# lcrekko/lq_mpc

Measured on AMD Instinct MI355X. Metric: MPC QP-steps/sec (batched systems) at n_x=4,n_u=2,N=10; 1/2/4/8 GPU, higher is better.
Workload: dtype f64

## Files before the change

### lq_mpc_amd/csrc/lqmpc_r16.hip

```cpp
#include <cstdio>
#include "lqmpc_r16_body.h"
#include "lqmpc_launch.h"

namespace lqmpc {

template <int NX, int NU, int N, int MODE, int LPI>
__global__ void __launch_bounds__(64, (R16Build<NX, NU, N, LPI>::WAVES)) lqmpc_r16_kernel(KParams p)
{
    using C = R16<NX, NU, N, LPI, (R16Build<NX, NU, N, LPI>::OCC == 2)>;
    __shared__ double lds_raw[C::IPW * C::INST];
    r16_body<NX, NU, N, MODE, LPI, R16Build<NX, NU, N, LPI>::OCC, (MODE == MODE_ROLLOUT && R16Build<NX, NU, N, LPI>::CHUNKS)>(p, lds_raw, (long long)blockIdx.x * C::IPW, p.Bsz);
}

template <int NX, int NU, int N, int LPI>
__global__ void __launch_bounds__(64, (R16Build<NX, NU, N, LPI>::WAVES)) lqmpc_r16_plan_kernel(KParams p)
{
    using C = R16<NX, NU, N, LPI, (R16Build<NX, NU, N, LPI>::OCC == 2)>;
    __shared__ double lds_raw[C::IPW * C::INST];
    r16_body<NX, NU, N, MODE_SOLVE, LPI, R16Build<NX, NU, N, LPI>::OCC, false, true>(p, lds_raw, (long long)blockIdx.x * C::IPW, p.Bsz);
}

template <int NX, int NU, int N, int LPI>
static void launch_r16_one(const KParams &p, hipStream_t stream)
{
    constexpr int IPW = 64 / LPI;
    const dim3 grid((unsigned)((p.Bsz + IPW - 1) / IPW));
    if (p.mode == MODE_SOLVE && p.Uplan) hipLaunchKernelGGL((lqmpc_r16_plan_kernel<NX, NU, N, LPI>), grid, dim3(64), 0, stream, p);
    else if (p.mode == MODE_SOLVE) hipLaunchKernelGGL((lqmpc_r16_kernel<NX, NU, N, MODE_SOLVE, LPI>), grid, dim3(64), 0, stream, p);
    else if (p.mode == MODE_MAXVN) hipLaunchKernelGGL((lqmpc_r16_kernel<NX, NU, N, MODE_MAXVN, LPI>), grid, dim3(64), 0, stream, p);
    else if (p.mode == MODE_SWEEP) hipLaunchKernelGGL((lqmpc_r16_kernel<NX, NU, N, MODE_SWEEP, LPI>), grid, dim3(64), 0, stream, p);
    else {
#ifdef LQMPC_R16_PROF
        long long z[36] = {0};
        (void)hipMemcpyToSymbol(HIP_SYMBOL(g_r16_prof), z, sizeof z);
#endif
        hipLaunchKernelGGL((lqmpc_r16_kernel<NX, NU, N, MODE_ROLLOUT, LPI>), grid, dim3(64), 0, stream, p);
#ifdef LQMPC_R16_PROF
        (void)hipStreamSynchronize(stream);
        (void)hipMemcpyFromSymbol(z, HIP_SYMBOL(g_r16_prof), sizeof z);
        fprintf(stderr, "r16 prof (block %d ticks): set-up on the matrix core %lld v_r %lld | rollout %lld\n", PROFBLK, z[5], z[6], z[7]);
        fprintf(stderr, "r16 prof (grid): waves %lld  set-up %.0f  total %.0f ticks/wave | free wave-steps %lld at %.0f ticks | busy wave-steps %lld at %.0f ticks, "
                "%.2f wave-iterations each (steps 1..T-1); %lld wave-iterations on the general (primal-capable) path in all\n", z[15], (double)z[13] / z[15], (double)z[14] / z[15], z[10], (double)z[8] / (z[10] ? z[10] : 1),
                z[11], (double)z[9] / (z[11] ? z[11] : 1), (double)z[12] / (z[11] ? z[11] : 1), z[16]);
        fprintf(stderr, "r16 prof (grid, ticks/wave): set-up on the matrix core %.0f v_r %.0f\n", (double)z[22] / z[15], (double)z[23] / z[15]);
        fprintf(stderr, "r16 prof (grid): %lld dual-only wave-iterations at %.0f ticks, %lld general at %.0f ticks\n", z[26], (double)z[24] / (z[26] ? z[26] : 1), z[16],
                (double)z[25] / (z[16] ? z[16] : 1));
        fprintf(stderr, "r16 prof (grid): step 0: %.0f ticks/wave, %.2f wave-iterations/wave, %.2f of them general; %lld of %lld wavefronts ever took the general (P-reading) path\n",
                (double)z[27] / z[15], (double)z[28] / z[15], (double)z[29] / z[15], z[30], z[15]);
        fprintf(stderr, "r16 prof (grid): chunks of iteration-free steps: %lld committed, %lld discarded with %lld steps computed for nothing (%.2f %% of the free wave-steps)\n",
                z[31], z[32], z[33], 100.0 * (double)z[33] / (z[10] ? z[10] : 1));
#endif
    }
}

#define R16E(NX, NU, N) {NX, NU, N, 16, "lqmpc_r16_kernel<" #NX "," #NU "," #N ">", launch_r16_one<NX, NU, N, 16>}
#define R64E(NX, NU, N) {NX, NU, N, 64, "lqmpc_r64_kernel<" #NX "," #NU "," #N ">", launch_r16_one<NX, NU, N, 64>}
static const ShapeEntry g_r16[] = {
    R16E(4, 2, 10),
    R16E(2, 1, 10),
    R16E(2, 1, 5), R16E(2, 1, 6), R16E(2, 1, 7), R16E(2, 1, 8), R16E(2, 1, 9),
    R16E(2, 1, 20), R16E(2, 1, 30),
    R64E(4, 2, 20),
};

// ... 22 lines not shown
```

### lq_mpc_amd/csrc/lqmpc_r16_body.h

```cpp
#pragma once
#include "lqmpc_wg_linalg.h"
#include "lqmpc_r16_setup.h"

namespace lqmpc {

using wg::ldsd;
using wg::ldsi;
using wg::rowb;
using wg::fmac_rowb;
using wg::fmac_rowb_self;
using wg::fmac_rowb4;
using wg::fmac_rowb_self4;
using wg::fmac_rowb_self2;
using wg::fmac_rowb_self3;
using wg::fmac_rowb_lanes4;
using wg::fmac_rowb_lanes4x2;
using wg::dpp_settle;

#ifdef LQMPC_R16_PROF
__device__ long long g_r16_prof[36];
#define RPROF(k) do { const long long now_ = clock64(); if (threadIdx.x == 0 && blockIdx.x == PROFBLK) g_r16_prof[k] += now_ - prof_t; if (k < 7) prof_ph[k] += now_ - prof_t; prof_t = clock64(); } while (0)
#define RPROF_START long long prof_t = clock64()
#define RPROF_ADD(k, v) do { if (threadIdx.x == 0) atomicAdd((unsigned long long *)&g_r16_prof[k], (unsigned long long)(v)); } while (0)
#ifndef PROFBLK
#define PROFBLK 0
#endif
#else
#define RPROF(k) do { } while (0)
#define RPROF_START do { } while (0)
#define RPROF_ADD(k, v) do { } while (0)
#endif

typedef unsigned long long mask_t;

template <int NX, int NU, int N, int LPI = 16, bool PACKED = false>
struct R16 {
    static constexpr int n = N * NU;
    static constexpr int RB = (n + LPI - 1) / LPI;
    static constexpr int IPW = 64 / LPI;
    static constexpr int CS = 4 * (((n + 1) / 2 + 3) / 4);
    static constexpr int LDW = n + 1;
    static constexpr int PK = PACKED ? n * (n + 1) / 2 : n * LDW;
    static constexpr int VEC = LPI * RB;
    static constexpr int oP = 0, oW = PK, oR = 2 * PK, oX = oR + VEC, oY = oX + VEC, oL = oY + VEC;
    static constexpr int oC = oL + CS / 2;
    static constexpr int CN0 = 3 * NX * NX + NU * NU + NX * NU;
    static constexpr int CN1 = (NX > NU ? NX : NU) * (2 * NX + 2 * NU);
    static constexpr int CN = CN0 > CN1 ? CN0 : CN1;
    static constexpr int oG = (NX > 8) ? oR : 0;
    static constexpr int SETUP = oG + n * NX;
    static constexpr int END = oC + CN + (CN & 1);
    static constexpr int oD = (END > SETUP) ? END : SETUP;
    static constexpr int INST = oD + 2;
    static constexpr int MAXIT = 12;
    static_assert(LPI == 16 || LPI == 64, "a DPP row or the whole wavefront");
    static_assert((n + 1) / 2 <= CS && n <= 64, "the smaller side must fit the gathered system");
};

template <int NX, int NU, int N, int LPI>
struct R16Build {
    static constexpr int OCC = ((LPI == 16 && N * NU > 10) || LPI == 64 || NX > 8) ? 2 : 1;
    static constexpr long long LDS_BYTES = (long long)(64 / LPI) * R16<NX, NU, N, LPI, (OCC == 2)>::INST * 8;
    static constexpr int WAVES = ((OCC == 2 || (N * NU <= 10 && LPI == 16)) && LDS_BYTES * 8 <= 160 * 1024) ? 2 : 1;
    static constexpr bool CHUNKS = NX == 4 && NU == 2 && ((LPI == 16 && N == 10) || (LPI == 64 && N == 20));
};

template <int LPI>
__device__ __forceinline__ mask_t iballot(bool c, int q)
{
    if constexpr (LPI == 16) return (__ballot(c) >> (16 * q)) & 0xFFFFull;
    else return __ballot(c);
}
template <int LPI>
__device__ __forceinline__ double ibcast(double x, int k)
{
    if constexpr (LPI == 16) return rowb(x, k);
    else return wg::rdlane(x, k);
}
template <int LPI>
__device__ __forceinline__ void ifmac_self4(double *acc, double y, int k)
{
    if constexpr (LPI == 16) fmac_rowb_self4(acc[0], acc[1], acc[2], acc[3], y, k);
    else {
#pragma unroll
        for (int e = 0; e < 4; ++e) acc[e] = __builtin_fma(wg::rdlane(acc[e], k), y, acc[e]);
    }
}
template <int LPI, int K, int CS>
__device__ __forceinline__ void ifmac_self_tail(double (&S)[CS], double &rhs, double g)
{
    constexpr int r = K % 4;
    if constexpr (LPI == 16) {
        if constexpr (r == 0) fmac_rowb_self4(S[K + 1], S[K + 2], S[K + 3], rhs, g, K);
        else if constexpr (r == 1) fmac_rowb_self3(S[K + 1], S[K + 2], rhs, g, K);
        else if constexpr (r == 2) fmac_rowb_self2(S[K + 1], rhs, g, K);
        else fmac_rowb_self(rhs, g, K);
    } else {
#pragma unroll
        for (int j = K + 1; j < 4 * (K / 4) + 4; ++j) S[j] = __builtin_fma(wg::rdlane(S[j], K), g, S[j]);
        rhs = __builtin_fma(wg::rdlane(rhs, K), g, rhs);
    }
}
template <int LPI>
__device__ __forceinline__ void isettle(double &x)
{
    if constexpr (LPI == 16) dpp_settle(x);
}
__device__ __forceinline__ int rowb_i(int x, int c)
{
    switch (c) {
#define LQMPC_X(C) case C: return __builtin_amdgcn_update_dpp(0, x, 0x150 + C, 0xF, 0xF, true);
        LQMPC_ROWB_CASES(LQMPC_X)
#undef LQMPC_X
    }
    return x;
}
__device__ __forceinline__ unsigned row_or(unsigned x)
{
    x |= (unsigned)__builtin_amdgcn_update_dpp(0, (int)x, 0x128, 0xF, 0xF, false);
    x |= (unsigned)__builtin_amdgcn_update_dpp(0, (int)x, 0x124, 0xF, 0xF, false);
    x |= (unsigned)__builtin_amdgcn_update_dpp(0, (int)x, 0x122, 0xF, 0xF, false);
    x |= (unsigned)__builtin_amdgcn_update_dpp(0, (int)x, 0x121, 0xF, 0xF, false);
    return x;
}
__device__ __forceinline__ unsigned row_umax(unsigned x)
{
    x = max(x, (unsigned)__builtin_amdgcn_update_dpp(0, (int)x, 0x128, 0xF, 0xF, false));
    x = max(x, (unsigned)__builtin_amdgcn_update_dpp(0, (int)x, 0x124, 0xF, 0xF, false));
    x = max(x, (unsigned)__builtin_amdgcn_update_dpp(0, (int)x, 0x122, 0xF, 0xF, false));
    x = max(x, (unsigned)__builtin_amdgcn_update_dpp(0, (int)x, 0x121, 0xF, 0xF, false));
    return x;
}

template <int NX, int NU, int N, int MODE, int LPI = 16, int OCC = 1, bool CHUNKS = false, bool PLAN = false>
__device__ __forceinline__ void r16_body(const KParams &p, double *lds_raw, long long slot0, long long slot_end)
{
    constexpr bool PACKED = (OCC == 2);
    using C = R16<NX, NU, N, LPI, PACKED>;
    constexpr int CS = C::CS;
    constexpr int n = C::n, RB = C::RB, LDW = C::LDW;
    constexpr int REC = NX * NX + NX * NU + NX;
    const int lane = threadIdx.x, q = lane / LPI, i = lane % LPI;
    ldsd *L = (ldsd *)lds_raw + q * C::INST;
    ldsd *Pp = L + C::oP, *Wp = L + C::oW, *rL = L + C::oR, *xL = L + C::oX, *yL = L + C::oY;
    ldsi *list = (ldsi *)(L + C::oL);
    const long long Bsz = p.Bsz;
    const long long b_raw = slot0 + q;
    const bool valid = b_raw < slot_end;
    const long long slot = valid ? b_raw : slot_end - 1;
    const long long b = p.perm ? (long long)p.perm[slot] : slot;
    const double *sh = p.sh;
    const mask_t nmask = (n == 64) ? ~0ull : ((1ull << n) - 1ull);

    int rw[RB], tri[RB];
    bool vrow[RB];
#pragma unroll
    for (int s = 0; s < RB; ++s) {
        rw[s] = i + LPI * s;
        tri[s] = rw[s] * (rw[s] + 1) / 2;
        vrow[s] = rw[s] < n;
    }

    auto ad = [&](int r, int tr, int j) -> int { if constexpr (PACKED) return (j <= r) ? tr + j : j * (j + 1) / 2 + r; else return r * LDW + j; };
    auto ad2 = [&](int a, int b2) -> int {
        if constexpr (PACKED) { const int hi = a > b2 ? a : b2, lo = a > b2 ? b2 : a; return hi * (hi + 1) / 2 + lo; }
        else return a * LDW + b2;
    };

    double G[RB][NX], vr[RB];
    constexpr bool CTL_F = MODE == MODE_CTL_FACTOR, CTL_S = MODE == MODE_CTL_STEP, CTL_R = MODE == MODE_CTL_ROLL;
    constexpr bool CTL_REC = CTL_S || CTL_R;
    using CR = CtlRecT<NX, NU, N>;
    constexpr bool LAZY_P = (LPI == 64 && !CTL_F) || CTL_REC;
    bool P_ready = !LAZY_P;
    bool W_ready = !CTL_REC;
    bool face_stays = false;
    auto tri_rc = [](int e, int &r, int &c) {
        r = (int)((__builtin_sqrtf(8.0f * (float)e + 1.0f) - 1.0f) * 0.5f);
        r = ((r + 1) * (r + 2) / 2 <= e) ? r + 1 : r;
        r = (r * (r + 1) / 2 > e) ? r - 1 : r;
        c = e - r * (r + 1) / 2;
    };
#ifdef LQMPC_NO_ROLL
    constexpr bool ROLL = false;
#else
    constexpr bool ROLL = LPI == 16 && NX <= 8 && N * ((NX + 3) / 4) <= 12 && MODE != MODE_MAXVN && !CTL_F && !CTL_REC;
#endif
    unsigned cold32[2] = {0u, 0u};
    bool cold_armed = false;
#ifdef LQMPC_R16_PROF
    const long long prof_t0 = clock64();
    int prof_wit = 0, prof_slow = 0, prof_fast = 0;
    long long prof_slowt = 0;
    long long prof_ph[8] = {0, 0, 0, 0, 0, 0, 0, 0};
#endif
    if constexpr (CTL_REC) {
        const double *rc = p.ctl_rec + b * p.ctl_stride;
#pragma unroll
        for (int s = 0; s < RB; ++s) {
            const int mr = vrow[s] ? rw[s] : 0;
#pragma unroll
            for (int a = 0; a < NX; ++a) G[s][a] = rc[CR::oG + mr * NX + a];
            vr[s] = vrow[s] ? rc[CR::oV + mr] : 0.0;
        }
    } else {
        RPROF_START;
        long long bg = b;
        ldsd *Lg = L;
        if constexpr (LPI == 16) {
            const int gq = (lane >> 2) & 3;
            const long long sraw = slot0 + gq, sl = sraw < slot_end ? sraw : slot_end - 1;
            bg = p.perm ? (long long)p.perm[sl] : sl;
            Lg = (ldsd *)lds_raw + gq * C::INST;
        }
        if constexpr (NX > 8) {
            static_assert(LPI == 16 && C::oG >= 2 * C::PK, "wide states: four instances per wavefront, G handed over behind P and W");
            r16_setup_wide<NX, NU, N, PACKED, RB>(setup_args(p), bg, Lg, C::oW, C::oG, C::oD);
#pragma unroll
            for (int s = 0; s < RB; ++s) {
#pragma unroll
                for (int a = 0; a < NX; ++a) {
                    const double x = L[C::oG + (vrow[s] ? rw[s] * NX + a : 0)];
                    G[s][a] = vrow[s] ? x : 0.0;
                }
            }
            __syncthreads();
        } else r16_setup_mfma<NX, NU, N, LPI, PACKED, RB, ROLL>(setup_args(p), bg, Lg, L, C::oW, C::oG, C::oD, G, roll_args(p), cold32[0], cold32[1]);
        if constexpr (!LAZY_P) r16_build_P<NX, NU, N, LPI, PACKED>(setup_args(p), bg, Lg, C::oP, C::oD);
        RPROF(5);
        const bool has_lin = p.has_lin != 0;
#pragma unroll
        for (int s = 0; s < RB; ++s) vr[s] = 0.0;
        if (has_lin) {
            if (p.has_ref) {
                double qr[RB];
#pragma unroll
                for (int s = 0; s < RB; ++s) qr[s] = 0.0;
                constexpr bool WIDE = NX > 8;
                double lam[NX], A2[WIDE ? 1 : NX][WIDE ? 1 : NX], B2[WIDE ? 1 : NX][WIDE ? 1 : NU];
                if constexpr (WIDE) {
                    const int ia = i < NX ? i : 0;
                    double Ac[NX], Bc[RB][NX];
#pragma unroll
                    for (int c = 0; c < NX; ++c) {
                        lam[c] = 0.0;
                        Ac[c] = p.rec ? p.rec[b * REC + c * NX + ia] : p.A[(long long)(c * NX + ia) * Bsz + b];
#pragma unroll
                        for (int s = 0; s < RB; ++s)
                            Bc[s][c] = p.rec ? p.rec[b * REC + NX * NX + c * NU + rw[s] % NU] : p.B[(long long)(c * NU + rw[s] % NU) * Bsz + b];
                    }
#pragma unroll 1
                    for (int r = N - 1; r >= 0; --r) {
                        const int oQ = (r < N - 1) ? p.so.Q : p.so.P;
                        double t = 0.0;
#pragma unroll
                        for (int c = 0; c < NX; ++c) t = __builtin_fma(sh[oQ + ia * NX + c], -sh[p.so.xref + c * N + r], t);
#pragma unroll
                        for (int c = 0; c < NX; ++c) t = __builtin_fma(Ac[c], lam[c], t);
                        yL[i] = t;
                        __syncthreads();
#pragma unroll
                        for (int a = 0; a < NX; ++a) lam[a] = yL[a];
                        __syncthreads();
#pragma unroll
                        for (int s = 0; s < RB; ++s) {
                            const int ui = rw[s] % NU;
                            double tk = 0.0;
#pragma unroll
                            for (int a = 0; a < NX; ++a) tk = __builtin_fma(Bc[s][a], lam[a], tk);
#pragma unroll
                            for (int j = 0; j < NU; ++j) tk = __builtin_fma(-sh[p.so.R + ui * NU + j], sh[p.so.uref + j * N + r], tk);
                            qr[s] = (vrow[s] && rw[s] / NU == r) ? 2.0 * tk : qr[s];
                        }
                    }
                } else {
#pragma unroll
                    for (int a = 0; a < NX; ++a) {
                        lam[a] = 0.0;
#pragma unroll
                        for (int c = 0; c < NX; ++c) A2[a][c] = p.rec ? p.rec[b * REC + a * NX + c] : p.A[(long long)(a * NX + c) * Bsz + b];
#pragma unroll
// ... 66 lines not shown
            }
        }
        RPROF(6);
    }
    if constexpr (CTL_F) {
        __syncthreads();
        const long long ir = p.ctl_idx ? (long long)p.ctl_idx[b] : b;
        if (valid && (unsigned long long)ir < (unsigned long long)p.ctl_n) {
            double *rc = p.ctl_rec + ir * p.ctl_stride;
            for (int e = i; e < NX * NX; e += LPI) rc[CR::oA + e] = p.A[(long long)e * Bsz + b];
            for (int e = i; e < NX * NU; e += LPI) rc[CR::oB + e] = p.B[(long long)e * Bsz + b];
#pragma unroll
            for (int s = 0; s < RB; ++s) {
                if (vrow[s]) {
#pragma unroll
                    for (int a = 0; a < NX; ++a) rc[CR::oG + rw[s] * NX + a] = G[s][a];
                    rc[CR::oV + rw[s]] = vr[s];
                }
            }
            for (int e = i; e < CR::tri; e += LPI) {
                int r, c;
                tri_rc(e, r, c);
                rc[CR::oW + e] = Wp[ad2(r, c)];
                rc[CR::oP + e] = Pp[ad2(r, c)];
            }
        }
        return;
    }
    auto ctl_fill = [&](ldsd *M, int off, bool on) {
        const double *src = p.ctl_rec + b * p.ctl_stride + off;
        constexpr int CNT = (CR::tri + LPI - 1) / LPI;
        double val[CNT];
#pragma unroll
        for (int k = 0; k < CNT; ++k) { const int e = i + LPI * k; val[k] = (on && e < CR::tri) ? src[e] : 0.0; }
#pragma unroll
        for (int k = 0; k < CNT; ++k) {
            const int e = i + LPI * k;
            if (on && e < CR::tri) {
                if constexpr (PACKED) M[e] = val[k];
                else { int r, c; tri_rc(e, r, c); M[r * LDW + c] = val[k]; M[c * LDW + r] = val[k]; }
            }
        }
        __syncthreads();
    };
    RPROF_START;
    RPROF_ADD(13, clock64() - prof_t0);

    long long bq = b;
    asm volatile("" : "+v"(bq));
    double h[RB], ctr[RB];
#pragma unroll
    for (int s = 0; s < RB; ++s) {
        const int k = rw[s] % NU;
        h[s] = vrow[s] ? 0.5 * (sh[p.so.ub + k] - sh[p.so.lb + k]) : 1.0;
        ctr[s] = vrow[s] ? 0.5 * (sh[p.so.ub + k] + sh[p.so.lb + k]) : 0.0;
    }
    double Qm[NX][NX], Rm[NU][NU];
    ldsd *cQ = L + C::oC, *cR = cQ + NX * NX;
    if constexpr (MODE == MODE_ROLLOUT || CTL_R) {
    } else if constexpr (OCC == 2) {
        if constexpr (NX > 8) {
            for (int e = i; e < NX * NX; e += LPI) cQ[e] = sh[p.so.Q + e];
            for (int e = i; e < NU * NU; e += LPI) cR[e] = sh[p.so.R + e];
        } else if (i == 0) {
#pragma unroll
            for (int a = 0; a < NX; ++a) {
#pragma unroll
                for (int c = 0; c < NX; ++c) {
                    cQ[a * NX + c] = sh[p.so.Q + a * NX + c];
                }
            }
#pragma unroll
            for (int k = 0; k < NU; ++k)
#pragma unroll
                for (int j = 0; j < NU; ++j) cR[k * NU + j] = sh[p.so.R + k * NU + j];
        }
        __syncthreads();
    } else {
#pragma unroll
        for (int a = 0; a < NX; ++a) {
#pragma unroll
            for (int c = 0; c < NX; ++c) Qm[a][c] = sh[p.so.Q + a * NX + c];
        }
#pragma unroll
        for (int k = 0; k < NU; ++k)
#pragma unroll
            for (int j = 0; j < NU; ++j) Rm[k][j] = sh[p.so.R + k * NU + j];
    }
    auto Qv = [&](int a, int c) -> double { if constexpr (OCC == 2) return cQ[a * NX + c]; else return Qm[a][c]; };
    auto Rv = [&](int k, int j) -> double { if constexpr (OCC == 2) return cR[k * NU + j]; else return Rm[k][j]; };
    const bool writer = valid && i == 0;
    mask_t pL = 0, pU = 0;
    int iters = 0, status = 0;
    auto qp = [&](const double (&x)[NX], double (&v)[RB]) {
        double vu[RB];
        mask_t cl = 0, cu = 0;
        bool bad = false;
#pragma unroll
        for (int s = 0; s < RB; ++s) {
            double acc = vr[s];
#pragma unroll
            for (int a = 0; a < NX; ++a) acc = __builtin_fma(G[s][a], x[a], acc);
            vu[s] = acc; v[s] = acc;
            cl |= iballot<LPI>(vrow[s] && acc < -h[s], q) << (LPI * s);
            cu |= iballot<LPI>(vrow[s] && acc > h[s], q) << (LPI * s);
            bad = bad || (vrow[s] && !(fabs(acc) < 1e300));
        }
        const bool rowbad = iballot<LPI>(bad, q) != 0;
// ... 711 lines not shown
            if (p.VN || (PLAN && p.Xplan)) vn = value_fn(x, v);
            stage_input(v, 0, u);
            if constexpr (PLAN) { if (p.Uplan) plan_rows(v); }
            if (writer) {
                fc[0] = pL; fc[1] = pU;
#pragma unroll
                for (int a = 0; a < NX; ++a) {
                    double xn = 0.0;
#pragma unroll
                    for (int cc = 0; cc < NX; ++cc) xn = __builtin_fma(Av(a, cc), x[cc], xn);
#pragma unroll
                    for (int k = 0; k < NU; ++k) xn = __builtin_fma(Bv(a, k), u[k], xn);
                    fc[2 + a] = (unsigned long long)__double_as_longlong(x[a]);
                    fc[2 + NX + a] = (unsigned long long)__double_as_longlong(xn);
                }
                if (p.VN) p.VN[b] = vn;
#pragma unroll
                for (int k = 0; k < NU; ++k) p.u0[(long long)k * Bsz + bq] = u[k];
            }
        } else if (MODE == MODE_SOLVE) {
            double x[NX], v[RB], u[NU];
#pragma unroll
            for (int a = 0; a < NX; ++a) x[a] = p.rec ? p.rec[bq * REC + NX * NX + NX * NU + a] : p.x0[(long long)a * Bsz + bq];
            cold_armed = ROLL;
            qp(x, v);
            const double vn = value_fn(x, v);
            stage_input(v, 0, u);
            if constexpr (PLAN) { if (p.Uplan) plan_rows(v); }
            if (writer) {
                p.VN[b] = vn;
#pragma unroll
                for (int k = 0; k < NU; ++k) p.u0[(long long)k * Bsz + bq] = u[k];
            }
        } else {
            double best = -1e308;
            for (int kk = 0; kk < p.K; ++kk) {
                double x[NX], v[RB];
#pragma unroll
                for (int a = 0; a < NX; ++a) x[a] = sh[p.so.x0s + a * p.K + kk];
                pL = 0; pU = 0;
                qp(x, v);
                const double vn = value_fn(x, v);
                best = (vn > best || vn != vn) ? vn : best;
            }
            if (writer) p.MV[b] = best;
        }
    }
    if (MODE == MODE_ROLLOUT || MODE == MODE_SWEEP || CTL_R) {
        pL = 0; pU = 0;
        double x[NX];
#pragma unroll
        for (int a = 0; a < NX; ++a) {
            if constexpr (CTL_R) x[a] = p.x0[(long long)a * Bsz + bq];
            else x[a] = p.rec ? p.rec[bq * REC + NX * NX + NX * NU + a] : p.x0[(long long)a * Bsz + bq];
        }
        int ia = i < NX ? i : 0, ik = i < NU ? i : 0;
        asm volatile("" : "+v"(ia), "+v"(ik));
        double Qr_[NX], Ar_[NX], Br_[NU], Rr_[NU];
#pragma unroll
        for (int c = 0; c < NX; ++c) {
            Qr_[c] = sh[p.so.Q + ia * NX + c];
            Ar_[c] = p.true_per_instance ? p.At[(long long)(ia * NX + c) * Bsz + bq] : sh[p.so.At + ia * NX + c];
        }
#pragma unroll
        for (int k = 0; k < NU; ++k) {
            Br_[k] = p.true_per_instance ? p.Bt[(long long)(ia * NU + k) * Bsz + bq] : sh[p.so.Bt + ia * NU + k];
            Rr_[k] = sh[p.so.R + ik * NU + k];
        }
        constexpr bool ROWS_IN_LDS = OCC == 2 && LPI == 64 && 2 * NX + 2 * NU > 12;
        constexpr int RW = 2 * NX + 2 * NU;
        static_assert((NX > NU ? NX : NU) * RW <= C::CN + (C::CN & 1), "the per-lane rows fit the constants region");
        ldsd *myc = L + C::oC + ((i < NX || i < NU) ? i : 0) * RW;
        if constexpr (ROWS_IN_LDS) {
            __syncthreads();
            if (i < NX || i < NU) {
#pragma unroll
                for (int c = 0; c < NX; ++c) { myc[c] = Ar_[c]; myc[NX + NU + c] = Qr_[c]; }
#pragma unroll
                for (int k = 0; k < NU; ++k) { myc[NX + k] = Br_[k]; myc[2 * NX + NU + k] = Rr_[k]; }
            }
            __syncthreads();
        }
        auto Ar = [&](int c) -> double { if constexpr (ROWS_IN_LDS) return myc[c]; else return Ar_[c]; };
        auto Br = [&](int k) -> double { if constexpr (ROWS_IN_LDS) return myc[NX + k]; else return Br_[k]; };
        auto Qr = [&](int c) -> double { if constexpr (ROWS_IN_LDS) return myc[NX + NU + c]; else return Qr_[c]; };
        auto Rr = [&](int k) -> double { if constexpr (ROWS_IN_LDS) return myc[2 * NX + NU + k]; else return Rr_[k]; };
        double costx, costu = 0.0;
        {
            double xm = x[0], qx = 0.0;
#pragma unroll
            for (int a = 1; a < NX; ++a) xm = (i == a) ? x[a] : xm;
#pragma unroll
            for (int c = 0; c < NX; ++c) qx = __builtin_fma(Qr(c), x[c], qx);
            costx = xm * qx;
        }
        if (p.X && writer) {
#pragma unroll
            for (int a = 0; a < NX; ++a) p.X[((long long)a * (p.T + 1)) * Bsz + bq] = x[a];
        }
#ifdef LQMPC_R16_PROF
        long long prof_ts = 0, prof_acc[5] = {0, 0, 0, 0, 0};
        int prof_nst = 1;
#endif
        constexpr int FREE_KMAX = 8;
        const bool free_chunks = CHUNKS && !p.X && !p.U;
        bool prev_free = false, chunk_hold = false;
        mask_t rows_mask[RB];
#pragma unroll
        for (int s = 0; s < RB; ++s) rows_mask[s] = __ballot(vrow[s]);
        for (int t = 0; t < p.T; ++t) {
            double v[RB], u[NU], xn[NX];
#ifdef LQMPC_R16_PROF
            if (t == 1) { RPROF_ADD(27, clock64() - prof_ts); RPROF_ADD(28, prof_wit); RPROF_ADD(29, prof_slow); }
            if (t > 0) {
                const long long d_ = clock64() - prof_ts;
                if (prof_wit) { prof_acc[1] += d_; prof_acc[3] += 1; prof_acc[4] += prof_wit; } else { prof_acc[0] += d_; prof_acc[2] += prof_nst; }
            }
            prof_ts = clock64();
            prof_wit = 0;
            prof_nst = 1;
// ... 119 lines not shown
```

### lq_mpc_amd/csrc/lqmpc_r16_setup.h

```cpp
#pragma once
#include "lqmpc_wg_linalg.h"

namespace lqmpc {

constexpr int SETUP_MAX_NX = 16, SETUP_MAX_NU = 4;

__device__ __forceinline__ double mm4(double a, double b, double c = 0.0) { return __builtin_amdgcn_mfma_f64_4x4x4f64(a, b, c, 0, 0, 0); }

template <int NX, int NU, int N, int LPI>
struct SetupT {
    static_assert(NX >= 1 && NX <= SETUP_MAX_NX, "state matrices are at most 4 x 4 tiles of 4 x 4");
    static_assert(NU >= 1 && NU <= SETUP_MAX_NU, "stage blocks of 1..4 rows");
    static constexpr int TX = (NX + 3) / 4;
    static constexpr int NUP = (NU == 3) ? 4 : NU;
    static constexpr int n = N * NU, npad = N * NUP;
    static constexpr int NT = (npad + 3) / 4;
    static constexpr int SPT = 4 / NUP;
    static constexpr int NTM = (LPI == 16) ? NT : (NT + 3) / 4;
    static constexpr bool EXACT_TILES = (NUP == NU) && (n % 4 == 0);
    static constexpr int tile_of_stage(int j) { return (j * NUP) / 4; }
    static constexpr int off_of_stage(int j) { return (j * NUP) % 4; }
    static constexpr bool live(int I, int j) { return ((I + 1) * SPT < N ? (I + 1) * SPT : N) - 1 > j; }
    __device__ static __forceinline__ int row_of(int rp) { return (rp < npad && rp % NUP < NU) ? (rp / NUP) * NU + rp % NUP : -1; }
};
// ... 175 lines not shown
        const double x = ld.S(p.oR, rr, cc, NU);
        Rd = (rr >= 0 && rr < NU && cc >= 0 && cc < NU) ? x : Rd;
    }
    double X[TX];
#pragma unroll
    for (int a = 0; a < TX; ++a) X[a] = Bpl[0][a];
    sfor<0, NT>([&](auto Dc) {
        constexpr int D = decltype(Dc)::value;
        double acc[NTM];
#pragma unroll
        for (int m = 0; m < NTM; ++m) acc[m] = (D == 0) ? Rd : 0.0;
        sfor<0, SPT>([&](auto pc) {
            constexpr int pp = decltype(pc)::value;
            constexpr int d = D * SPT + pp;
            if constexpr (d > 0) {
                double Xn[TX];
#pragma unroll
                for (int a = 0; a < TX; ++a) {
                    double v = (d <= SPT - 1) ? Bpl[d <= SPT - 1 ? d : 0][a] : 0.0;
#pragma unroll
                    for (int k2 = 0; k2 < TX; ++k2) v = mm4(At[k2][a], X[k2], v);
                    Xn[a] = v;
                }
#pragma unroll
                for (int a = 0; a < TX; ++a) X[a] = Xn[a];
            }
            if constexpr (LPI == 16) {
                sfor<D, NT>([&](auto Ic) {
                    constexpr int I = decltype(Ic)::value;
#pragma unroll
                    for (int k2 = 0; k2 < TX; ++k2) acc[I] = mm4(ap[I][pp][k2], X[k2], acc[I]);
                });
            } else {
                sfor<D / 4, NTM>([&](auto mc) {
                    constexpr int m = decltype(mc)::value;
#pragma unroll
                    for (int k2 = 0; k2 < TX; ++k2) acc[m] = mm4(ap[m][pp][k2], X[k2], acc[m]);
                });
            }
        });
        if constexpr (LPI == 16) {
            sfor<D, NT>([&](auto Ic) { constexpr int I = decltype(Ic)::value; store_tile<T, PACKED>(Pp, dP, I, I - D, 2.0 * acc[I], true, r, c); });
        } else {
            sfor<D / 4, NTM>([&](auto mc) {
                constexpr int m = decltype(mc)::value;
                const int I = 4 * m + g;
                store_tile<T, PACKED>(Pp, dP, I, I - D, 2.0 * acc[m], I >= D && I < NT, r, c);
            });
        }
    });
    __syncthreads();
}

template <int NX, int NU, int N, int LPI, bool PACKED, int RB, bool ROLL = false, bool READ_G = true>
__device__ __forceinline__ void r16_setup_mfma(const SetupArgs &p, long long bg, wg::ldsd *Lg, wg::ldsd *Lq, int oW, int oG, int oD,
                                              double (&G)[RB][NX], const RollArgs &ra, unsigned &coldL, unsigned &coldU)
{
    static_assert(!ROLL || (LPI == 16 && N * NU <= 32), "the cold-start roll serves the four-instance mapping");
    static_assert(READ_G || !ROLL, "the roll runs under the read-back of G");
    using T = SetupT<NX, NU, N, LPI>;
    constexpr int n = T::n, NT = T::NT, SPT = T::SPT, NTM = T::NTM, TX = T::TX, NUP = T::NUP;
    const int lane = threadIdx.x, r = lane >> 4, c = lane & 3, g = (lane >> 2) & 3;
    wg::ldsd *Wp = Lg + oW, *Gs = Lg + oG;
    const int dW = oD - oW, dG = oD - oG;
    const ModelLd<NX, NU> ld(p, bg);
    double A[TX][TX], Q[TX][TX], S[TX][TX];
    double Bp[TX], nBt[TX];
    double Bpl[SPT][TX], nBpl[SPT][TX];
#pragma unroll
    for (int a = 0; a < TX; ++a) {
#pragma unroll
        for (int b = 0; b < TX; ++b) {
            A[a][b] = ld.A(4 * a + r, 4 * b + c);
            Q[a][b] = ld.S(p.oQ, 4 * a + r, 4 * b + c, NX); S[a][b] = ld.S(p.oP, 4 * a + r, 4 * b + c, NX);
        }
        Bp[a] = ld.B(4 * a + r, c); nBt[a] = -ld.B(4 * a + c, r);
#pragma unroll
        for (int qq = 0; qq < SPT; ++qq) { Bpl[qq][a] = ld.B(4 * a + r, c - qq * NUP); nBpl[qq][a] = -Bpl[qq][a]; }
    }
    const double Rp = (r == c && r >= NU && r < NUP) ? 1.0 : ld.S(p.oR, r, c, NU);

    double Wacc[(LPI == 16) ? NTM : 1][(LPI == 16) ? NT : 1];
    wg::d4_t Wb[(LPI == 64) ? NTM * (NTM + 1) / 2 : 1];
    double rho[NTM][TX];
    double TtA[NTM], TDA[NTM], Dh = 0.0;
    double KT[ROLL ? N : 1][TX];
#pragma unroll
    for (int m = 0; m < NTM; ++m) {
        TDA[m] = 0.0; TtA[m] = 0.0;
#pragma unroll
        for (int a = 0; a < TX; ++a) rho[m][a] = 0.0;
        if constexpr (LPI == 16) {
#pragma unroll
            for (int J = 0; J < NT; ++J) Wacc[m][J] = 0.0;
        }
    }
    if constexpr (LPI == 64) {
#pragma unroll
        for (int e = 0; e < NTM * (NTM + 1) / 2; ++e) Wb[e] = wg::d4_t{0.0, 0.0, 0.0, 0.0};
    }
    auto advance = [&](double (&o)[TX], const double (&Acl)[TX][TX], const double (&add)[TX], bool with_add) {
        double t[TX];
#pragma unroll
        for (int a = 0; a < TX; ++a) {
            double v = with_add ? add[a] : 0.0;
#pragma unroll
            for (int k = 0; k < TX; ++k) v = mm4(Acl[k][a], o[k], v);
            t[a] = v;
        }
#pragma unroll
        for (int a = 0; a < TX; ++a) o[a] = t[a];
    };
    auto dotc = [&](const double (&x)[TX], const double (&o)[TX], double cc) -> double {
        double v = cc;
#pragma unroll
        for (int k = 0; k < TX; ++k) v = mm4(x[k], o[k], v);
        return v;
    };
    sfor<0, N>([&](auto jc) {
        constexpr int j = N - 1 - decltype(jc)::value;
        constexpr int Ij = T::tile_of_stage(j), off = T::off_of_stage(j), q = off / NUP;
        constexpr bool first_of_tile = (j == N - 1) || (q == SPT - 1);
        double SA[TX][TX], SB[TX], F[TX], K[TX], Acl[TX][TX], Ktp[TX];
#pragma unroll
        for (int a = 0; a < TX; ++a) {
#pragma unroll
            for (int b = 0; b < TX; ++b) {
                double v = 0.0;
#pragma unroll
                for (int k = 0; k < TX; ++k) v = mm4(S[k][a], A[k][b], v);
                SA[a][b] = v;
            }
            double w = 0.0;
#pragma unroll
            for (int k = 0; k < TX; ++k) w = mm4(S[k][a], Bp[k], w);
            SB[a] = w;
        }
        double Re = Rp;
#pragma unroll
        for (int k = 0; k < TX; ++k) Re = mm4(Bp[k], SB[k], Re);
#pragma unroll
        for (int b = 0; b < TX; ++b) {
            double v = 0.0;
#pragma unroll
            for (int k = 0; k < TX; ++k) v = mm4(Bp[k], SA[k][b], v);
            F[b] = v;
        }
        const double R0 = small_inverse<NUP, true>(Re, r, c);
#pragma unroll
        for (int b = 0; b < TX; ++b) K[b] = mm4(R0, F[b]);
        if constexpr (ROLL && off != 0) {
#pragma unroll
            for (int b = 0; b < TX; ++b) KT[j][b] = mm4(F[b], R0);
        }
#pragma unroll
        for (int a = 0; a < TX; ++a)
#pragma unroll
            for (int b = 0; b < TX; ++b) Acl[a][b] = mm4(nBt[a], K[b], A[a][b]);
        if constexpr (j > 0) {
            double Zm[TX][TX];
#pragma unroll
            for (int a = 0; a < TX; ++a)
#pragma unroll
                for (int b = 0; b < TX; ++b) {
                    double v = 0.0;
#pragma unroll
                    for (int k = 0; k < TX; ++k) v = mm4(S[k][a], Acl[k][b], v);
                    Zm[a][b] = v;
                }
#pragma unroll
            for (int a = 0; a < TX; ++a)
#pragma unroll
                for (int b = 0; b < TX; ++b) {
                    double v = Q[a][b];
#pragma unroll
                    for (int k = 0; k < TX; ++k) v = mm4(A[k][a], Zm[k][b], v);
// ... 40 lines not shown
            constexpr int m0 = Ij / 4;
            sfor<m0, NTM>([&](auto mc) {
                constexpr int m = decltype(mc)::value;
                const bool mine = (4 * m + g == Ij);
                TtA[m] = dotc(nBpl[q], rho[m], (first_of_tile ? 0.0 : TtA[m]) + (mine ? Iq : 0.0));
            });
            if constexpr (q == 0) {
                sfor<m0, NTM>([&](auto mc) { constexpr int m = decltype(mc)::value; TDA[m] = mm4(Dh, TtA[m]); });
                sfor<m0, NTM>([&](auto mc) {
                    constexpr int m = decltype(mc)::value;
                    sfor<m0, m + 1>([&](auto nc) {
                        constexpr int m2 = decltype(nc)::value;
                        Wb[m * (m + 1) / 2 + m2] = __builtin_amdgcn_mfma_f64_16x16x4f64(TDA[m], TtA[m2], Wb[m * (m + 1) / 2 + m2], 0, 0, 0);
                    });
                });
            }
            sfor<m0, NTM>([&](auto mc) {
                constexpr int m = decltype(mc)::value;
                const bool mine = (4 * m + g == Ij);
                double add[TX];
#pragma unroll
                for (int a = 0; a < TX; ++a) add[a] = mine ? Ktp[a] : 0.0;
                advance(rho[m], Acl, add, true);
            });
        }
    });

#pragma unroll
    for (int m = 0; m < NTM; ++m) {
        const int I = (LPI == 16) ? m : 4 * m + g;
        const int row = T::row_of(4 * I + c);
#pragma unroll
        for (int a = 0; a < TX; ++a) Gs[(4 * a + r < NX && row >= 0) ? row * NX + 4 * a + r : dG] = -rho[m][a];
    }
    if constexpr (READ_G) {
        __syncthreads();
        const int i = lane % LPI;
        const wg::ldsd *Gq = Lq + oG;
#pragma unroll
        for (int s = 0; s < RB; ++s) {
            const int row = i + LPI * s;
#pragma unroll
            for (int a = 0; a < NX; ++a) {
                const double x = Gq[row < n ? row * NX + a : 0];
                G[s][a] = row < n ? x : 0.0;
            }
        }
        __syncthreads();
    }

    coldL = 0u; coldU = 0u;
    if constexpr (ROLL) {
        unsigned bL = 0u, bU = 0u;
        if (ra.roll) {
            constexpr int REC = NX * NX + NX * NU + NX;
            const double I4 = (r == c) ? 1.0 : 0.0;
            double At[TX][TX], xr[TX];
#pragma unroll
            for (int a = 0; a < TX; ++a) {
#pragma unroll
                for (int b = 0; b < TX; ++b) At[b][a] = mm4(A[a][b], I4);
                const bool v = c == 0 && 4 * a + r < NX;
                const int ia = v ? 4 * a + r : 0;
                const double x = p.rec ? p.rec[bg * REC + NX * NX + NX * NU + ia] : ra.x0[(long long)ia * p.Bsz + bg];
                xr[a] = v ? x : 0.0;
            }
            const int kk = r < NU ? r : 0;
            const double hk = (r < NU) ? 0.5 * (p.sh[ra.oUb + kk] - p.sh[ra.oLb + kk]) : 1.0;
            const unsigned one = (c == 0 && r < NU) ? (1u << r) : 0u;
            sfor<0, N>([&](auto jc) {
                constexpr int j = decltype(jc)::value;
                double kx = 0.0;
#pragma unroll
                for (int b = 0; b < TX; ++b) kx = mm4(KT[j][b], xr[b], kx);
                double xn[TX];
                if constexpr (j + 1 < N) {
#pragma unroll
                    for (int a = 0; a < TX; ++a) {
                        double v = 0.0;
#pragma unroll
                        for (int b = 0; b < TX; ++b) v = mm4(At[b][a], xr[b], v);
                        xn[a] = v;
                    }
                }
                bL |= (kx > hk) ? (one << (j * NU)) : 0u;
                bU |= (kx < -hk) ? (one << (j * NU)) : 0u;
                const double un = fmin(fmax(kx, -hk), hk);
                if constexpr (j + 1 < N) {
#pragma unroll
                    for (int a = 0; a < TX; ++a) xr[a] = mm4(nBt[a], un, xn[a]);
                }
            });
        }
        unsigned mLq[4], mUq[4];
#pragma unroll
        for (int gq = 0; gq < 4; ++gq) {
            mLq[gq] = 0u; mUq[gq] = 0u;
#pragma unroll
            for (int k = 0; k < NU; ++k) {
                mLq[gq] |= (unsigned)__builtin_amdgcn_readlane((int)bL, 16 * k + 4 * gq);
                mUq[gq] |= (unsigned)__builtin_amdgcn_readlane((int)bU, 16 * k + 4 * gq);
            }
        }
        coldL = r == 0 ? mLq[0] : (r == 1 ? mLq[1] : (r == 2 ? mLq[2] : mLq[3]));
        coldU = r == 0 ? mUq[0] : (r == 1 ? mUq[1] : (r == 2 ? mUq[2] : mUq[3]));
    }

    if constexpr (LPI == 16) {
#pragma unroll
        for (int I = 0; I < NT; ++I)
#pragma unroll
            for (int J = 0; J <= I; ++J) store_tile<T, PACKED>(Wp, dW, I, J, Wacc[I][J], true, r, c);
    } else {
        constexpr int LDW = n + 1;
#pragma unroll
        for (int m = 0; m < NTM; ++m)
#pragma unroll
            for (int m2 = 0; m2 <= m; ++m2)
#pragma unroll
                for (int e = 0; e < 4; ++e) {
                    const int row = T::row_of(16 * m + (lane >> 4) + 4 * e), col = T::row_of(16 * m2 + (lane & 15));
                    const bool low = row >= 0 && col >= 0 && col <= row;
                    const double val = Wb[m * (m + 1) / 2 + m2][e];
                    if constexpr (PACKED) Wp[low ? row * (row + 1) / 2 + col : dW] = val;
                    else {
                        Wp[low ? row * LDW + col : dW] = val;
                        Wp[(low && col < row) ? col * LDW + row : dW] = val;
                    }
                }
    }
    __syncthreads();
}

template <int NX, int NU, int N, bool PACKED, int RB>
__device__ __attribute__((noinline)) void r16_setup_wide(const SetupArgs p, long long bg, wg::ldsd *Lg, int oW, int oG, int oD)
{
    double G[RB][NX];
    unsigned cl, cu;
    r16_setup_mfma<NX, NU, N, 16, PACKED, RB, false, false>(p, bg, Lg, Lg, oW, oG, oD, G, RollArgs{nullptr, 0, 0, 0}, cl, cu);
}

}
```

Measured before the change: 7.739 billion.

## Load per-instance inputs in one round and build P inside the MFMA set-up

For the n_x=4,n_u=2,N=10 rollout path, shared Q/R/P-weight loads are issued before the permutation lookup resolves, and the per-instance A, B, x0 and box bounds are parked in LDS once. Later phases read them from LDS instead of reloading from global memory. The separate r16_build_P pass is replaced by computing the condensed Hessian P on the matrix-core path during the Riccati/roll sweep, reusing the already loaded A and B. This aims to cut repeated global loads and a separate set-up pass, at the cost of extra register pressure (Lt, ap arrays) and an unconditional roll computation.

After: 7.912 billion, median of 6. +2.2%, better.

```diff
diff --git a/lq_mpc_amd/csrc/lqmpc_r16.hip b/lq_mpc_amd/csrc/lqmpc_r16.hip
--- a/lq_mpc_amd/csrc/lqmpc_r16.hip
+++ b/lq_mpc_amd/csrc/lqmpc_r16.hip
@@ -9,7 +9,8 @@
 {
     using C = R16<NX, NU, N, LPI, (R16Build<NX, NU, N, LPI>::OCC == 2)>;
     __shared__ double lds_raw[C::IPW * C::INST];
-    r16_body<NX, NU, N, MODE, LPI, R16Build<NX, NU, N, LPI>::OCC, (MODE == MODE_ROLLOUT && R16Build<NX, NU, N, LPI>::CHUNKS)>(p, lds_raw, (long long)blockIdx.x * C::IPW, p.Bsz);
+    r16_body<NX, NU, N, MODE, LPI, R16Build<NX, NU, N, LPI>::OCC, (MODE == MODE_ROLLOUT && R16Build<NX, NU, N, LPI>::CHUNKS), false,
+             (MODE == MODE_ROLLOUT && R16Build<NX, NU, N, LPI>::ONE_TRIP)>(p, lds_raw, (long long)blockIdx.x * C::IPW, p.Bsz);
 }
 
 template <int NX, int NU, int N, int LPI>
diff --git a/lq_mpc_amd/csrc/lqmpc_r16_body.h b/lq_mpc_amd/csrc/lqmpc_r16_body.h
--- a/lq_mpc_amd/csrc/lqmpc_r16_body.h
+++ b/lq_mpc_amd/csrc/lqmpc_r16_body.h
@@ -63,6 +63,7 @@
     static constexpr long long LDS_BYTES = (long long)(64 / LPI) * R16<NX, NU, N, LPI, (OCC == 2)>::INST * 8;
     static constexpr int WAVES = ((OCC == 2 || (N * NU <= 10 && LPI == 16)) && LDS_BYTES * 8 <= 160 * 1024) ? 2 : 1;
     static constexpr bool CHUNKS = NX == 4 && NU == 2 && ((LPI == 16 && N == 10) || (LPI == 64 && N == 20));
+    static constexpr bool ONE_TRIP = NX == 4 && NU == 2 && LPI == 16 && N == 10;
 };
 
 template <int LPI>
@@ -132,7 +133,7 @@
     return x;
 }
 
-template <int NX, int NU, int N, int MODE, int LPI = 16, int OCC = 1, bool CHUNKS = false, bool PLAN = false>
+template <int NX, int NU, int N, int MODE, int LPI = 16, int OCC = 1, bool CHUNKS = false, bool PLAN = false, bool ONE_TRIP = false>
 __device__ __forceinline__ void r16_body(const KParams &p, double *lds_raw, long long slot0, long long slot_end)
 {
     constexpr bool PACKED = (OCC == 2);
@@ -140,6 +141,7 @@
     constexpr int CS = C::CS;
     constexpr int n = C::n, RB = C::RB, LDW = C::LDW;
     constexpr int REC = NX * NX + NX * NU + NX;
+    constexpr int PK_RW = 2 * NX + 2 * NU, PK_X = (NX > NU ? NX : NU) * PK_RW;
     const int lane = threadIdx.x, q = lane / LPI, i = lane % LPI;
     ldsd *L = (ldsd *)lds_raw + q * C::INST;
     ldsd *Pp = L + C::oP, *Wp = L + C::oW, *rL = L + C::oR, *xL = L + C::oX, *yL = L + C::oY;
@@ -148,7 +150,10 @@
     const long long b_raw = slot0 + q;
     const bool valid = b_raw < slot_end;
     const long long slot = valid ? b_raw : slot_end - 1;
-    const long long b = p.perm ? (long long)p.perm[slot] : slot;
+    int b_perm = 0;
+    if constexpr (ONE_TRIP) { if (p.perm) b_perm = p.perm[slot]; }
+    long long b = slot;
+    if constexpr (!ONE_TRIP) b = p.perm ? (long long)p.perm[slot] : slot;
     const double *sh = p.sh;
     const mask_t nmask = (n == 64) ? ~0ull : ((1ull << n) - 1ull);
 
@@ -210,7 +215,8 @@
         if constexpr (LPI == 16) {
             const int gq = (lane >> 2) & 3;
             const long long sraw = slot0 + gq, sl = sraw < slot_end ? sraw : slot_end - 1;
-            bg = p.perm ? (long long)p.perm[sl] : sl;
+            if constexpr (ONE_TRIP) bg = sl;
+            else bg = p.perm ? (long long)p.perm[sl] : sl;
             Lg = (ldsd *)lds_raw + gq * C::INST;
         }
         if constexpr (NX > 8) {
@@ -225,8 +231,50 @@
                 }
             }
             __syncthreads();
+        } else if constexpr (ONE_TRIP) {
+            static_assert(MODE == MODE_ROLLOUT && LPI == 16 && ROLL && !LAZY_P, "one round of loads: the rollout of the four-instance mapping");
+            static_assert(PK_X + NX + 2 * NU <= C::CN + (C::CN & 1) && NX + 2 * NU <= LPI, "the parked values fit the constants region, one per lane");
+            const int ia = i < NX ? i : 0, ik = i < NU ? i : 0, eb = i - NX;
+            const bool tpi = p.true_per_instance != 0, isbox = eb >= 0 && eb < 2 * NU;
+            double rowv[PK_RW];
+#pragma unroll
+            for (int c = 0; c < NX; ++c) rowv[NX + NU + c] = sh[p.so.Q + ia * NX + c];
+#pragma unroll
+            for (int k = 0; k < NU; ++k) rowv[2 * NX + NU + k] = sh[p.so.R + ik * NU + k];
+            if (!tpi) {
+#pragma unroll
+                for (int c = 0; c < NX; ++c) rowv[c] = sh[p.so.At + ia * NX + c];
+#pragma unroll
+                for (int k = 0; k < NU; ++k) rowv[NX + k] = sh[p.so.Bt + ia * NU + k];
+            }
+            const double boxv = sh[isbox ? (eb < NU ? p.so.lb + eb : p.so.ub + eb - NU) : p.so.lb];
+            auto late_bg = [&]() -> long long {
+                if (!p.perm) return bg;
+                const int bi = b_perm;
+                b = (long long)b_perm;
+                const int b0 = __builtin_amdgcn_readlane(bi, 0), b1 = __builtin_amdgcn_readlane(bi, 16);
+                const int b2 = __builtin_amdgcn_readlane(bi, 32), b3 = __builtin_amdgcn_readlane(bi, 48);
+                const int gq = (lane >> 2) & 3;
+                return (long long)(gq == 0 ? b0 : (gq == 1 ? b1 : (gq == 2 ? b2 : b3)));
+            };
+            auto late_park = [&]() {
+                if (tpi) {
+#pragma unroll
+                    for (int c = 0; c < NX; ++c) rowv[c] = p.At[(long long)(ia * NX + c) * Bsz + b];
+#pragma unroll
+                    for (int k = 0; k < NU; ++k) rowv[NX + k] = p.Bt[(long long)(ia * NU + k) * Bsz + b];
+                }
+                const double x0v = p.rec ? p.rec[b * REC + NX * NX + NX * NU + ia] : p.x0[(long long)ia * Bsz + b];
+                ldsd *pk = L + C::oC;
+                const bool own = i < NX || i < NU;
+#pragma unroll
+                for (int e = 0; e < PK_RW; ++e) pk[own ? i * PK_RW + e : C::oD - C::oC] = rowv[e];
+                pk[(i < NX || isbox) ? PK_X + i : C::oD - C::oC] = i < NX ? x0v : boxv;
+            };
+            const LateT<decltype(late_bg), decltype(late_park)> late{late_bg, late_park};
+            r16_setup_mfma<NX, NU, N, LPI, PACKED, RB, ROLL, true, true>(setup_args(p), bg, Lg, L, C::oW, C::oG, C::oD, G, roll_args(p), cold32[0], cold32[1], C::oP, late);
         } else r16_setup_mfma<NX, NU, N, LPI, PACKED, RB, ROLL>(setup_args(p), bg, Lg, L, C::oW, C::oG, C::oD, G, roll_args(p), cold32[0], cold32[1]);
-        if constexpr (!LAZY_P) r16_build_P<NX, NU, N, LPI, PACKED>(setup_args(p), bg, Lg, C::oP, C::oD);
+        if constexpr (!LAZY_P && !ONE_TRIP) r16_build_P<NX, NU, N, LPI, PACKED>(setup_args(p), bg, Lg, C::oP, C::oD);
         RPROF(5);
         const bool has_lin = p.has_lin != 0;
 #pragma unroll
@@ -399,8 +447,14 @@
 #pragma unroll
     for (int s = 0; s < RB; ++s) {
         const int k = rw[s] % NU;
+        if constexpr (ONE_TRIP) {
+            const double lbk = L[C::oC + PK_X + NX + k], ubk = L[C::oC + PK_X + NX + NU + k];
+            h[s] = vrow[s] ? 0.5 * (ubk - lbk) : 1.0;
+            ctr[s] = vrow[s] ? 0.5 * (ubk + lbk) : 0.0;
+        } else {
         h[s] = vrow[s] ? 0.5 * (sh[p.so.ub + k] - sh[p.so.lb + k]) : 1.0;
         ctr[s] = vrow[s] ? 0.5 * (sh[p.so.ub + k] + sh[p.so.lb + k]) : 0.0;
+        }
     }
     double Qm[NX][NX], Rm[NU][NU];
     ldsd *cQ = L + C::oC, *cR = cQ + NX * NX;
@@ -1218,11 +1272,18 @@
 #pragma unroll
         for (int a = 0; a < NX; ++a) {
             if constexpr (CTL_R) x[a] = p.x0[(long long)a * Bsz + bq];
+            else if constexpr (ONE_TRIP) x[a] = L[C::oC + PK_X + a];
             else x[a] = p.rec ? p.rec[bq * REC + NX * NX + NX * NU + a] : p.x0[(long long)a * Bsz + bq];
         }
         int ia = i < NX ? i : 0, ik = i < NU ? i : 0;
         asm volatile("" : "+v"(ia), "+v"(ik));
         double Qr_[NX], Ar_[NX], Br_[NU], Rr_[NU];
+        if constexpr (ONE_TRIP) {
+#pragma unroll
+            for (int c = 0; c < NX; ++c) { Qr_[c] = L[C::oC + ia * PK_RW + NX + NU + c]; Ar_[c] = L[C::oC + ia * PK_RW + c]; }
+#pragma unroll
+            for (int k = 0; k < NU; ++k) { Br_[k] = L[C::oC + ia * PK_RW + NX + k]; Rr_[k] = L[C::oC + ik * PK_RW + 2 * NX + NU + k]; }
+        } else {
 #pragma unroll
         for (int c = 0; c < NX; ++c) {
             Qr_[c] = sh[p.so.Q + ia * NX + c];
@@ -1232,6 +1293,7 @@
         for (int k = 0; k < NU; ++k) {
             Br_[k] = p.true_per_instance ? p.Bt[(long long)(ia * NU + k) * Bsz + bq] : sh[p.so.Bt + ia * NU + k];
             Rr_[k] = sh[p.so.R + ik * NU + k];
+        }
         }
         constexpr bool ROWS_IN_LDS = OCC == 2 && LPI == 64 && 2 * NX + 2 * NU > 12;
         constexpr int RW = 2 * NX + 2 * NU;
diff --git a/lq_mpc_amd/csrc/lqmpc_r16_setup.h b/lq_mpc_amd/csrc/lqmpc_r16_setup.h
--- a/lq_mpc_amd/csrc/lqmpc_r16_setup.h
+++ b/lq_mpc_amd/csrc/lqmpc_r16_setup.h
@@ -251,21 +251,68 @@
     __syncthreads();
 }
 
-template <int NX, int NU, int N, int LPI, bool PACKED, int RB, bool ROLL = false, bool READ_G = true>
+struct NoLate {
+    __device__ __forceinline__ long long bg() const { return 0; }
+    __device__ __forceinline__ void park() const {}
+};
+template <class FB, class FP>
+struct LateT {
+    const FB &fb;
+    const FP &fp;
+    __device__ __forceinline__ long long bg() const { return fb(); }
+    __device__ __forceinline__ void park() const { fp(); }
+};
+template <int NX, int NU, int N, int LPI, bool PACKED, int RB, bool ROLL = false, bool READ_G = true, bool ONE_TRIP = false, class Late = NoLate>
 __device__ __forceinline__ void r16_setup_mfma(const SetupArgs &p, long long bg, wg::ldsd *Lg, wg::ldsd *Lq, int oW, int oG, int oD,
-                                              double (&G)[RB][NX], const RollArgs &ra, unsigned &coldL, unsigned &coldU)
+                                              double (&G)[RB][NX], const RollArgs &ra, unsigned &coldL, unsigned &coldU, int oP = 0,
+                                              const Late &late = Late())
 {
     static_assert(!ROLL || (LPI == 16 && N * NU <= 32), "the cold-start roll serves the four-instance mapping");
     static_assert(READ_G || !ROLL, "the roll runs under the read-back of G");
+    static_assert(!ONE_TRIP || (ROLL && LPI == 16), "one round of loads: the four-instance mapping with the roll");
     using T = SetupT<NX, NU, N, LPI>;
     constexpr int n = T::n, NT = T::NT, SPT = T::SPT, NTM = T::NTM, TX = T::TX, NUP = T::NUP;
     const int lane = threadIdx.x, r = lane >> 4, c = lane & 3, g = (lane >> 2) & 3;
     wg::ldsd *Wp = Lg + oW, *Gs = Lg + oG;
     const int dW = oD - oW, dG = oD - oG;
-    const ModelLd<NX, NU> ld(p, bg);
     double A[TX][TX], Q[TX][TX], S[TX][TX];
     double Bp[TX], nBt[TX];
     double Bpl[SPT][TX], nBpl[SPT][TX];
+    double Rp;
+    double Rd = 0.0, hk1 = 1.0, x0r[TX];
+    if constexpr (ONE_TRIP) {
+        const ModelLd<NX, NU> sl(p, 0);
+#pragma unroll
+        for (int a = 0; a < TX; ++a)
+#pragma unroll
+            for (int b = 0; b < TX; ++b) { Q[a][b] = sl.S(p.oQ, 4 * a + r, 4 * b + c, NX); S[a][b] = sl.S(p.oP, 4 * a + r, 4 * b + c, NX); }
+        Rp = (r == c && r >= NU && r < NUP) ? 1.0 : sl.S(p.oR, r, c, NU);
+#pragma unroll
+        for (int qq = 0; qq < SPT; ++qq) {
+            const int rr = r - qq * NUP, cc = c - qq * NUP;
+            const double x = sl.S(p.oR, rr, cc, NU);
+            Rd = (rr >= 0 && rr < NU && cc >= 0 && cc < NU) ? x : Rd;
+        }
+        const int kk = r < NU ? r : 0;
+        hk1 = (r < NU) ? 0.5 * (p.sh[ra.oUb + kk] - p.sh[ra.oLb + kk]) : 1.0;
+        const long long bgl = late.bg();
+        const ModelLd<NX, NU> ld(p, bgl);
+        constexpr int REC = NX * NX + NX * NU + NX;
+#pragma unroll
+        for (int a = 0; a < TX; ++a) {
+#pragma unroll
+            for (int b = 0; b < TX; ++b) A[a][b] = ld.A(4 * a + r, 4 * b + c);
+            Bp[a] = ld.B(4 * a + r, c); nBt[a] = -ld.B(4 * a + c, r);
+#pragma unroll
+            for (int qq = 0; qq < SPT; ++qq) { Bpl[qq][a] = ld.B(4 * a + r, c - qq * NUP); nBpl[qq][a] = -Bpl[qq][a]; }
+            const bool v = c == 0 && 4 * a + r < NX;
+            const int ia = v ? 4 * a + r : 0;
+            const double x = p.rec ? p.rec[bgl * REC + NX * NX + NX * NU + ia] : ra.x0[(long long)ia * p.Bsz + bgl];
+            x0r[a] = v ? x : 0.0;
+        }
+        late.park();
+    } else {
+    const ModelLd<NX, NU> ld(p, bg);
 #pragma unroll
     for (int a = 0; a < TX; ++a) {
 #pragma unroll
@@ -277,7 +324,15 @@
 #pragma unroll
         for (int qq = 0; qq < SPT; ++qq) { Bpl[qq][a] = ld.B(4 * a + r, c - qq * NUP); nBpl[qq][a] = -Bpl[qq][a]; }
     }
-    const double Rp = (r == c && r >= NU && r < NUP) ? 1.0 : ld.S(p.oR, r, c, NU);
+    Rp = (r == c && r >= NU && r < NUP) ? 1.0 : ld.S(p.oR, r, c, NU);
+    }
+    double Lt[TX][TX], ap[ONE_TRIP ? NTM : 1][SPT][TX];
+    if constexpr (ONE_TRIP) {
+#pragma unroll
+        for (int a = 0; a < TX; ++a)
+#pragma unroll
+            for (int b = 0; b < TX; ++b) Lt[a][b] = S[a][b];
+    }
 
     double Wacc[(LPI == 16) ? NTM : 1][(LPI == 16) ? NT : 1];
     wg::d4_t Wb[(LPI == 64) ? NTM * (NTM + 1) / 2 : 1];
@@ -321,6 +376,37 @@
         constexpr int Ij = T::tile_of_stage(j), off = T::off_of_stage(j), q = off / NUP;
         constexpr bool first_of_tile = (j == N - 1) || (q == SPT - 1);
         double SA[TX][TX], SB[TX], F[TX], K[TX], Acl[TX][TX], Ktp[TX];
+        if constexpr (ONE_TRIP) {
+            constexpr int Ip = j / SPT, pp = j % SPT;
+#pragma unroll
+            for (int a = 0; a < TX; ++a) {
+                double v = 0.0;
+#pragma unroll
+                for (int k2 = 0; k2 < TX; ++k2) v = mm4(Lt[k2][a], Bpl[pp][k2], v);
+                ap[Ip][pp][a] = v;
+            }
+            if constexpr (j > 0) {
+                double LA[TX][TX];
+#pragma unroll
+                for (int a = 0; a < TX; ++a)
+#pragma unroll
+                    for (int b = 0; b < TX; ++b) {
+                        double v = 0.0;
+#pragma unroll
+                        for (int k2 = 0; k2 < TX; ++k2) v = mm4(Lt[k2][a], A[k2][b], v);
+                        LA[a][b] = v;
+                    }
+#pragma unroll
+                for (int a = 0; a < TX; ++a)
+#pragma unroll
+                    for (int b = 0; b < TX; ++b) {
+                        double v = Q[a][b];
+#pragma unroll
+                        for (int k2 = 0; k2 < TX; ++k2) v = mm4(A[k2][a], LA[k2][b], v);
+                        Lt[a][b] = v;
+                    }
+            }
+        }
 #pragma unroll
         for (int a = 0; a < TX; ++a) {
 #pragma unroll
@@ -467,21 +553,27 @@
     coldL = 0u; coldU = 0u;
     if constexpr (ROLL) {
         unsigned bL = 0u, bU = 0u;
-        if (ra.roll) {
+        double At[TX][TX];
+        if (ONE_TRIP || ra.roll) {
             constexpr int REC = NX * NX + NX * NU + NX;
             const double I4 = (r == c) ? 1.0 : 0.0;
-            double At[TX][TX], xr[TX];
+            double xr[TX];
 #pragma unroll
             for (int a = 0; a < TX; ++a) {
 #pragma unroll
                 for (int b = 0; b < TX; ++b) At[b][a] = mm4(A[a][b], I4);
+                if constexpr (ONE_TRIP) xr[a] = x0r[a];
+                else {
                 const bool v = c == 0 && 4 * a + r < NX;
                 const int ia = v ? 4 * a + r : 0;
                 const double x = p.rec ? p.rec[bg * REC + NX * NX + NX * NU + ia] : ra.x0[(long long)ia * p.Bsz + bg];
                 xr[a] = v ? x : 0.0;
+                }
             }
             const int kk = r < NU ? r : 0;
-            const double hk = (r < NU) ? 0.5 * (p.sh[ra.oUb + kk] - p.sh[ra.oLb + kk]) : 1.0;
+            double hk;
+            if constexpr (ONE_TRIP) hk = hk1;
+            else hk = (r < NU) ? 0.5 * (p.sh[ra.oUb + kk] - p.sh[ra.oLb + kk]) : 1.0;
             const unsigned one = (c == 0 && r < NU) ? (1u << r) : 0u;
             sfor<0, N>([&](auto jc) {
                 constexpr int j = decltype(jc)::value;
@@ -505,6 +597,42 @@
 #pragma unroll
                     for (int a = 0; a < TX; ++a) xr[a] = mm4(nBt[a], un, xn[a]);
                 }
+            });
+            if constexpr (ONE_TRIP) { bL = ra.roll ? bL : 0u; bU = ra.roll ? bU : 0u; }
+        }
+        if constexpr (ONE_TRIP) {
+            wg::ldsd *Pp = Lg + oP;
+            const int dP = oD - oP;
+            double X[TX];
+#pragma unroll
+            for (int a = 0; a < TX; ++a) X[a] = Bpl[0][a];
+            sfor<0, NT>([&](auto Dc) {
+                constexpr int D = decltype(Dc)::value;
+                double acc[NTM];
+#pragma unroll
+                for (int m = 0; m < NTM; ++m) acc[m] = (D == 0) ? Rd : 0.0;
+                sfor<0, SPT>([&](auto pc) {
+                    constexpr int pp = decltype(pc)::value;
+                    constexpr int d = D * SPT + pp;
+                    if constexpr (d > 0) {
+                        double Xn[TX];
+#pragma unroll
+                        for (int a = 0; a < TX; ++a) {
+                            double v = (d <= SPT - 1) ? Bpl[d <= SPT - 1 ? d : 0][a] : 0.0;
+#pragma unroll
+                            for (int k2 = 0; k2 < TX; ++k2) v = mm4(At[k2][a], X[k2], v);
+                            Xn[a] = v;
+                        }
+#pragma unroll
+                        for (int a = 0; a < TX; ++a) X[a] = Xn[a];
+                    }
+                    sfor<D, NT>([&](auto Ic) {
+                        constexpr int I = decltype(Ic)::value;
+#pragma unroll
+                        for (int k2 = 0; k2 < TX; ++k2) acc[I] = mm4(ap[I][pp][k2], X[k2], acc[I]);
+                    });
+                });
+                sfor<D, NT>([&](auto Ic) { constexpr int I = decltype(Ic)::value; store_tile<T, PACKED>(Pp, dP, I, I - D, 2.0 * acc[I], true, r, c); });
             });
         }
         unsigned mLq[4], mUq[4];
```
